# Parskatt/RoMa

Hardware: AMD Instinct MI355X
Metric: image-pairs/sec, roma_outdoor 560->864, batch=8 per GPU (higher is better)
Workload: dtype bf16; 1 GPU; roma_outdoor match() 560->864, symmetric, upsample_preds, 8 pairs/GPU/step, seeded synthetic weights + N(0,1) images; precision policy of the reference's bf16 timing script: bfloat16 DINOv2 + float16 autocast for VGG / decoder / refiners (ROMA_MIXED), f32 accumulate; precision_policy=mixed, global_batch=8, streams_per_gpu=2, parallelism=single GPU, outputs_finite=True

## Files before the change

### roma_amd/csrc/api.hip

```cpp
#include <algorithm>
#include <mutex>
#include <map>
#include <vector>
#include <dlfcn.h>
#include <string.h>

#include "../../include/roma_hip.h"
#include "attention.h"
#include "conv64.h"
#include "conv_patch.h"
#include "elementwise.h"
#include "gemm.h"
#include "local_corr.h"
#include "pool_proj.h"
#include "model.h"
#include "refiner_block.h"
#include "kde.h"
#include "keypoints.h"
#include "tiny.h"
#include "vit.h"
#include "sampling.h"
#include "essential.h"
#include "model_refine.h"
#include "pose_refine.h"
// ... 60 lines not shown

const char* roma_last_error(void) { return g_err.c_str(); }
const char* roma_version(void) { return "roma_hip 0.3 (gfx950, 16-bit storage = " ROMA_H16_NAME ")"; }
int roma_h16_format(void) { return ROMA_H16_CODE; }
int roma_abi_stamp(void) { return ROMA_ABI_VERSION * 100000 + (int)sizeof(roma_vit_args_t); }
int roma_self_check(void) { return roma::internal_h16_code(); }

int roma_create(const roma_config_t* cfg, roma_handle_t* out) {
  ROMA_REQUIRE(cfg && out, "roma_create: null argument");
  ROMA_REQUIRE(cfg->coarse_h > 0 && cfg->coarse_w > 0 && cfg->coarse_h % 14 == 0 && cfg->coarse_w % 14 == 0,
               "Needs to be multiple of 14 for backbone");
  ROMA_REQUIRE(cfg->coarse_h >= 16 && cfg->coarse_w >= 16, "roma_create: coarse resolution too small for the stride-16 pyramid");
  ROMA_REQUIRE(cfg->upsample_h >= 0 && cfg->upsample_w >= 0 && (cfg->upsample_h == 0 || (cfg->upsample_h >= 16 && cfg->upsample_w >= 16)),
               "roma_create: bad upsample resolution");
  ROMA_REQUIRE(cfg->max_batch >= 1, "roma_create: max_batch must be >= 1");
  if (cfg->precision == ROMA_MIXED) {
    ROMA_REQUIRE(ROMA_H16_CODE == ROMA_F16, "ROMA_MIXED: load libroma_hip_f16.so (it runs DINOv2 through libroma_hip.so)");
  } else if (dt_code(cfg->precision) < 0) {
    return ROMA_ERR_ARG;
  }
  int ndev = 0;
  ROMA_CHECK_HIP(hipGetDeviceCount(&ndev));
  ROMA_REQUIRE(cfg->device >= 0 && cfg->device < ndev, "roma_create: no such HIP device (the HIP path has no CPU fallback)");
  roma_model* h = new roma_model();
  h->m.cfg = *cfg;
  *out = h;
  return 0;
}

int roma_set_tensor(roma_handle_t h, const char* name, int ndim, const int64_t* shape, const void* data, int is_int64) {
  ROMA_REQUIRE(h, "roma_set_tensor: null handle");
  return h->m.set_tensor(name, ndim, shape, data, is_int64);
}

int roma_finalize(roma_handle_t h) {
  ROMA_REQUIRE(h, "roma_finalize: null handle");
  return h->m.finalize();
}

int roma_set_option(roma_handle_t h, const char* key, int value) {
  ROMA_REQUIRE(h && key, "roma_set_option: null argument");
  const std::string k(key);
  if (k == "symmetric") h->m.cfg.symmetric = value ? 1 : 0;
  else if (k == "upsample_preds") {
    ROMA_REQUIRE(!value || h->m.cfg.upsample_h > 0, "roma_set_option: handle was created without an upsample resolution");
    h->m.cfg.upsample_preds = value ? 1 : 0;
  } else if (k == "attenuate_cert") h->m.cfg.attenuate_cert = value ? 1 : 0;
  else if (k == "debug") h->m.debug = value != 0;
  else if (k == "fuse_refiner_blocks") h->m.fuse_refiner_blocks = value != 0;
  else if (k == "compose_out_conv") h->m.compose_out_conv = value != 0;
  else if (k == "vit_bf16_residual") h->m.vit_bf16_residual = value != 0;
  else if (k == "dual_stream") h->m.n_streams = value != 0 ? 2 : 1;
  else if (k == "trace") h->m.trace_on = value != 0;
  else if (k == "streams") {
    ROMA_REQUIRE(value >= 1 && value <= Model::MAX_STREAMS, "roma_set_option: streams must be 1..4");
    h->m.n_streams = value;
  }
  else {
    set_error("roma_set_option: unknown key " + k);
    return ROMA_ERR_ARG;
  }
  return 0;
}

int roma_set_option_f(roma_handle_t h, const char* key, double value) {
  ROMA_REQUIRE(h && key, "roma_set_option_f: null argument");
  const std::string k(key);
  if (k == "coarse_scale_factor") {
    ROMA_REQUIRE(value >= 0.0, "roma_set_option_f: coarse_scale_factor must be >= 0 (0 = derive from the handle's resolution)");
    h->m.coarse_scale_factor = value;
  } else {
    set_error("roma_set_option_f: unknown key " + k);
    return ROMA_ERR_ARG;
  }
  return 0;
}

int roma_match(roma_handle_t h, int B, const float* im_a, const float* im_b, const float* im_a_hr, const float* im_b_hr,
               float* warp_out, float* cert_out, void* stream) {
  ROMA_REQUIRE(h, "roma_match: null handle");
  return h->m.match(B, im_a, im_b, im_a_hr, im_b_hr, warp_out, cert_out, S(stream));
}

int roma_forward(roma_handle_t h, int B, const float* im_a, const float* im_b, const roma_forward_args_t* a, void* stream) {
  ROMA_REQUIRE(h, "roma_forward: null handle");
  return h->m.forward(B, im_a, im_b, a, S(stream));
}

long roma_debug_fetch(roma_handle_t h, const char* name, void* dst_host, long nbytes) {
  if (!h || !name) return ROMA_ERR_ARG;
  auto it = h->m.dbg.find(name);
  if (it == h->m.dbg.end()) {
    set_error(std::string("roma_debug_fetch: no such stage: ") + name);
    return ROMA_ERR_ARG;
  }
  if (!dst_host) return (long)it->second.second;
  if ((size_t)nbytes < it->second.second) {
    set_error("roma_debug_fetch: destination too small");
    return ROMA_ERR_ARG;
  }
  if (hipSetDevice(h->m.cfg.device) != hipSuccess || hipDeviceSynchronize() != hipSuccess) return ROMA_ERR_HIP;
  if (hipMemcpy(dst_host, it->second.first, it->second.second, hipMemcpyDeviceToHost) != hipSuccess) return ROMA_ERR_HIP;
  return (long)it->second.second;
}

int roma_debug_inject(roma_handle_t h, const char* name, const void* src_host, long nbytes) {
// ... 443 lines not shown
```

### roma_amd/csrc/model.h

```cpp
#pragma once
#include <stdlib.h>

#include <map>
#include <mutex>
#include <string>
#include <vector>

#include "../../include/roma_hip.h"
#include "common.h"

namespace roma {

extern std::mutex g_peer_mutex;

struct HostTensor {
  std::vector<int64_t> shape;
  std::vector<float> data;
  long numel() const {
    long n = 1;
    for (auto d : shape) n *= d;
    return n;
  }
};

// ... 47 lines not shown
    if (off > peak) peak = off;
    return p;
  }
  size_t mark() const { return off; }
  void release(size_t m) { off = m; }
};

class Model {
 public:
  static constexpr int MAX_STREAMS_DECL = 4;
  roma_config_t cfg{};
  int act_dt = 0;
  bool mixed = false;
  bool pack_as_bf16 = false;
  void* peer_lib = nullptr;
  int (*peer_vit_forward)(const roma_vit_args_t*, void*) = nullptr;
  bool finalized = false;
  bool debug = false;
  bool compose_out_conv = !(getenv("ROMA_COMPOSE_OUT") && atoi(getenv("ROMA_COMPOSE_OUT")) == 0);
  bool vgg_slab_major = !(getenv("ROMA_CONV_KORDER") && atoi(getenv("ROMA_CONV_KORDER")) == 0) &&
                        !(getenv("ROMA_CONV_PATCH") && atoi(getenv("ROMA_CONV_PATCH")) == 0);
  int vgg_korder[12] = {0};
  bool fuse_refiner_blocks = true;
  bool vit_bf16_residual = true;
  bool trace_on = false;
  static constexpr int TRACE_MAX = 1024;
  unsigned long long* trace_dev[MAX_STREAMS_DECL] = {nullptr};
  std::vector<std::string> trace_names[MAX_STREAMS_DECL];
  int trace_n[MAX_STREAMS_DECL] = {0};
  double coarse_scale_factor = 0.0;
  std::map<std::string, HostTensor> host;

  float *c1_w = nullptr, *c1_b = nullptr;
  Lin vgg[12];
  int vgg_cin[12] = {0}, vgg_cout[12] = {0};
  Lin patch;
  float *cls_tok = nullptr, *pos_emb = nullptr;
  VitBlockW dino[24];
  float *dino_nw = nullptr, *dino_nb = nullptr;
  VitBlockW tdec[5];
  Lin to_out;
  float *gp_w = nullptr, *gp_b = nullptr;
  Lin proj[5];
  RefinerW ref[5];

  Arena arena;
  Arena persist;
  static constexpr int MAX_STREAMS = 4;
  int n_streams = 2, streams_ready = 1;
  size_t side_arena_bytes = 0, side_persist_bytes = 0;
  Arena side_arena[MAX_STREAMS - 1], side_persist[MAX_STREAMS - 1];
  hipStream_t side[MAX_STREAMS - 1] = {nullptr};
  hipEvent_t ev_fork = nullptr, ev_join[MAX_STREAMS - 1] = {nullptr};
  std::vector<void*> owned;
  std::map<std::string, std::pair<void*, size_t>> dbg;
  int dbg_cur_slot = 0;
  std::map<std::string, std::pair<void*, size_t>> inject;
  int debug_inject(const char* name, const void* host, size_t bytes);

  ~Model();
  int set_tensor(const char* name, int ndim, const int64_t* shape, const void* data, int is_int64);
  int finalize();
  int match(int B, const float* ima, const float* imb, const float* ima_hr, const float* imb_hr, float* warp,
            float* cert, hipStream_t st);
  int forward(int B, const float* ima, const float* imb, const roma_forward_args_t* fw, hipStream_t st);

 private:
  int ensure_side_streams(int n);
  int match_streams(int B, const float* ima, const float* imb, const float* ima_hr, const float* imb_hr, float* warp,
                    float* cert, hipStream_t st);
  int check_contract();
  int pack_weights();
  int load_peer();
  int match_impl(int B, const float* ima, const float* imb, const float* ima_hr, const float* imb_hr, float* warp,
                 float* cert, hipStream_t st, bool dry, Arena& arena, Arena& persist, const roma_forward_args_t* fw = nullptr);
  int dbg_save(const char* name, const void* p, size_t bytes, hipStream_t st);
  template <typename F> int upload_f32(const std::vector<float>& v, F** out);
  int upload_act(const std::vector<float>& v, void** out);
  int make_lin(const std::vector<float>& w, const std::vector<float>* b, int N, int K, Lin* out);
};

int gp_posterior(const void* pf, long ldf, int act_dt, int B, bool symmetric, int th, int tw, const float* gp_w,
                 const float* gp_b, float* mu, long ld_mu, Arena& arena, hipStream_t st, bool dry);

int cholesky_solve_t(float* A, float* Rt, float* LT, float* Linv, float* LinvT, int n, int d, int batch, hipStream_t st,
                     long strideA = 0, long strideR = 0);

}
```

### roma_amd/csrc/model.hip

```cpp
#include "model.h"

#include <dlfcn.h>
#include <math.h>
#include <stdlib.h>
#include <string.h>

#include <algorithm>
#include <atomic>
#include <set>

#include "attention.h"
#include "conv64.h"
#include "pool_proj.h"
#include "elementwise.h"
#include "gemm.h"
#include "local_corr.h"
#include "refiner_block.h"
#include "vit.h"

namespace roma {

std::mutex g_peer_mutex;
extern void* g_peer_lib;
extern int g_mixed_handles;

static const int VGG_IDX[12] = {0, 3, 7, 10, 14, 17, 20, 23, 27, 30, 33, 36};
static const int VGG_CH[12] = {64, 64, 128, 128, 256, 256, 256, 256, 512, 512, 512, 512};
static const char* SCALES[5] = {"16", "8", "4", "2", "1"};
static const int SCALE_INT[5] = {16, 8, 4, 2, 1};
static const int PROJ_CIN[5] = {1024, 512, 256, 128, 64};
static const int PROJ_COUT[5] = {512, 512, 256, 64, 9};
static const int REF_EMB[5] = {128, 64, 32, 16, 6};
static const int REF_RAD[5] = {7, 3, 2, 0, 0};

Model::~Model() {
  for (int i = 0; i < MAX_STREAMS - 1; ++i) {
    if (side[i]) (void)hipStreamDestroy(side[i]);
    if (ev_join[i]) (void)hipEventDestroy(ev_join[i]);
  }
  if (ev_fork) (void)hipEventDestroy(ev_fork);
  for (void* p : owned) (void)hipFree(p);
  for (auto& kv : dbg) (void)hipFree(kv.second.first);
  for (auto& kv : inject) (void)hipFree(kv.second.first);
  if (peer_lib) {
    std::lock_guard<std::mutex> lk(g_peer_mutex);
    --g_mixed_handles;
  }
}


int Model::load_peer() {
  static void* lib = nullptr;
  static int (*fwd)(const roma_vit_args_t*, void*) = nullptr;
  std::lock_guard<std::mutex> lk(g_peer_mutex);
  if (!lib) {
    ROMA_REQUIRE(roma_h16_format() == ROMA_F16, "ROMA_MIXED is a mode of the binary16 build (libroma_hip_f16.so)");
    Dl_info info;
    ROMA_REQUIRE(dladdr(reinterpret_cast<void*>(&roma_vit_forward), &info) && info.dli_fname, "ROMA_MIXED: cannot locate this library");
    std::string path(info.dli_fname);
    const size_t slash = path.find_last_of('/');
    path = (slash == std::string::npos ? std::string("") : path.substr(0, slash + 1)) + "libroma_hip.so";
    void* l = dlopen(path.c_str(), RTLD_NOW | RTLD_LOCAL | RTLD_DEEPBIND);
    if (!l) {
      set_error("ROMA_MIXED: cannot load the bfloat16 library " + path + ": " + (dlerror() ? dlerror() : "?"));
      return ROMA_ERR_STATE;
    }
    auto fmt = reinterpret_cast<int (*)(void)>(dlsym(l, "roma_h16_format"));
    auto self = reinterpret_cast<int (*)(void)>(dlsym(l, "roma_self_check"));
    auto abi = reinterpret_cast<int (*)(void)>(dlsym(l, "roma_abi_stamp"));
    auto f = reinterpret_cast<int (*)(const roma_vit_args_t*, void*)>(dlsym(l, "roma_vit_forward"));
    std::string why;
    if (!fmt || !f || !self || !abi) why = "it does not export roma_h16_format / roma_self_check / roma_abi_stamp / roma_vit_forward (an older build)";
    else if (fmt() != ROMA_BF16) why = "it is not the bfloat16 build";
    else if (abi() != roma_abi_stamp()) why = "its ABI stamp " + std::to_string(abi()) + " differs from this library's " + std::to_string(roma_abi_stamp()) + " (stale build: roma_vit_args_t would be misread)";
    else if (self() != ROMA_BF16) why = "its internal calls resolve into another library (symbol interposition: link both builds with -Wl,-Bsymbolic)";
    if (!why.empty()) {
      dlclose(l);
      set_error("ROMA_MIXED: " + path + " cannot serve as the bfloat16 sibling: " + why);
      return ROMA_ERR_STATE;
    }
    lib = l;
    fwd = f;
    g_peer_lib = l;
  }
  if (!peer_lib) ++g_mixed_handles;
  peer_lib = lib;
  peer_vit_forward = fwd;
  return 0;
}

int Model::debug_inject(const char* name, const void* host, size_t bytes) {
  ROMA_REQUIRE(name, "roma_debug_inject: null name");
  const std::string k(name);
// ... 400 lines not shown
          for (int k = 0; k < r.Cp; ++k) {
            const float wv = cw[(size_t)o * r.Cp + k];
            const float hi = bf16_to_f32(f32_to_bf16(wv));
            hl[(size_t)o * r.Cp + k] = hi;
            hl[(size_t)(4 + o) * r.Cp + k] = wv - hi;
          }
          fb[o] = cb[o];
        }
        if (int rc = upload_act(hl, &r.ocf_w)) return rc;
        if (int rc = upload_f32(fb, &r.ocf_b)) return rc;
      }
    }
  }
  return 0;
}

int Model::finalize() {
  ROMA_REQUIRE(!finalized, "roma_finalize: already finalized");
  ROMA_CHECK_HIP(hipSetDevice(cfg.device));
  if (int rc = check_contract()) return rc;
  act_dt = cfg.precision == ROMA_F32 ? DT_F32 : DT_BF16;
  mixed = cfg.precision == ROMA_MIXED;
  if (mixed)
    if (int rc = load_peer()) return rc;
  if (int rc = pack_weights()) return rc;
  host.clear();
  arena.dry = persist.dry = true;
  arena.peak = persist.peak = 0;
  const int keep_sym = cfg.symmetric, keep_up = cfg.upsample_preds;
  cfg.symmetric = 1;
  cfg.upsample_preds = cfg.upsample_h > 0 ? 1 : 0;
  int rc = match_impl(cfg.max_batch, nullptr, nullptr, nullptr, nullptr, nullptr, nullptr, nullptr, true, arena, persist);
  Arena plan, plan_p;
  if (!rc && cfg.max_batch >= 2)
    rc = match_impl(cfg.max_batch / 2, nullptr, nullptr, nullptr, nullptr, nullptr, nullptr, nullptr, true, plan, plan_p);
  cfg.symmetric = keep_sym;
  cfg.upsample_preds = keep_up;
  if (rc) return rc;
  side_arena_bytes = plan.peak + 4096;
  side_persist_bytes = plan_p.peak + 4096;
  arena.cap = arena.peak + 4096;
  persist.cap = persist.peak + 4096;
  ROMA_CHECK_HIP(hipMalloc((void**)&arena.base, arena.cap));
  owned.push_back(arena.base);
  ROMA_CHECK_HIP(hipMalloc((void**)&persist.base, persist.cap));
  owned.push_back(persist.base);
  ROMA_CHECK_HIP(hipMemset(persist.base, 0, persist.cap));
  ROMA_CHECK_HIP(hipMemset(arena.base, 0, arena.cap));
  arena.dry = persist.dry = false;
  finalized = true;
  return 0;
}

int Model::ensure_side_streams(int n) {
  for (int i = streams_ready - 1; i + 1 < n; ++i) {
    Arena &a = side_arena[i], &p = side_persist[i];
    a.cap = side_arena_bytes;
    p.cap = side_persist_bytes;
    ROMA_CHECK_HIP(hipMalloc((void**)&a.base, a.cap));
    owned.push_back(a.base);
    ROMA_CHECK_HIP(hipMalloc((void**)&p.base, p.cap));
    owned.push_back(p.base);
    ROMA_CHECK_HIP(hipMemset(p.base, 0, p.cap));
    ROMA_CHECK_HIP(hipMemset(a.base, 0, a.cap));
    ROMA_CHECK_HIP(hipDeviceSynchronize());
    a.dry = p.dry = false;
    ROMA_CHECK_HIP(hipStreamCreateWithFlags(&side[i], hipStreamNonBlocking));
    ROMA_CHECK_HIP(hipEventCreateWithFlags(&ev_join[i], hipEventDisableTiming));
    if (!ev_fork) ROMA_CHECK_HIP(hipEventCreateWithFlags(&ev_fork, hipEventDisableTiming));
    streams_ready = i + 2;
  }
  return 0;
}

static const int g_dbg_dual_slot = getenv("ROMA_DEBUG_DUAL_SLOT") ? atoi(getenv("ROMA_DEBUG_DUAL_SLOT")) : -1;

int Model::dbg_save(const char* name, const void* p, size_t bytes, hipStream_t st) {
  if (!debug) return 0;
  if (g_dbg_dual_slot >= 0) {
    static const std::string only = std::string(",") + (getenv("ROMA_DEBUG_ONLY") ? getenv("ROMA_DEBUG_ONLY") : "") + ",";
    if (dbg_cur_slot != g_dbg_dual_slot || only.find(std::string(",") + name + ",") == std::string::npos) return 0;
  }
  auto it = dbg.find(name);
  if (it == dbg.end() || it->second.second != bytes) {
    if (it != dbg.end()) (void)hipFree(it->second.first);
    void* q = nullptr;
    ROMA_CHECK_HIP(hipMalloc(&q, bytes));
    dbg[name] = {q, bytes};
    it = dbg.find(name);
  }
  ROMA_CHECK_HIP(hipMemcpyAsync(it->second.first, p, bytes, hipMemcpyDeviceToDevice, st));
  return 0;
}

int Model::match(int B, const float* ima, const float* imb, const float* ima_hr, const float* imb_hr, float* warp,
                 float* cert, hipStream_t st) {
  ROMA_REQUIRE(finalized, "roma_match: call roma_finalize first");
  ROMA_REQUIRE(B >= 1 && B <= cfg.max_batch, "roma_match: batch size out of range (max_batch)");
  ROMA_REQUIRE(ima && imb && warp && cert, "roma_match: null image / output pointer");
  if (cfg.upsample_preds) {
    ROMA_REQUIRE(cfg.upsample_h > 0, "roma_match: upsample_preds set but the handle has no upsample resolution");
    ROMA_REQUIRE(ima_hr && imb_hr, "roma_match: upsample_preds requires im_A_high_res and im_B_high_res");
  }
  ROMA_CHECK_HIP(hipSetDevice(cfg.device));
  return match_streams(B, ima, imb, ima_hr, imb_hr, warp, cert, st);
}

int Model::forward(int B, const float* ima, const float* imb, const roma_forward_args_t* fw, hipStream_t st) {
  ROMA_REQUIRE(finalized, "roma_forward: call roma_finalize first");
  ROMA_REQUIRE(B >= 1 && B <= cfg.max_batch, "roma_forward: batch size out of range (max_batch)");
  ROMA_REQUIRE(ima && imb && fw, "roma_forward: null image / argument pointer");
  if (fw->upsample) {
    ROMA_REQUIRE(cfg.upsample_h > 0, "roma_forward: upsample pass on a handle without an upsample resolution");
    ROMA_REQUIRE(fw->seed_flow && fw->seed_cert && fw->seed_h > 0 && fw->seed_w > 0,
                 "roma_forward: the upsample pass needs batch[\"corresps\"] (seed_flow / seed_cert)");
  }
  ROMA_CHECK_HIP(hipSetDevice(cfg.device));
  return match_impl(B, ima, imb, nullptr, nullptr, nullptr, nullptr, st, false, arena, persist, fw);
}

int Model::match_streams(int B, const float* ima, const float* imb, const float* ima_hr, const float* imb_hr, float* warp,
                         float* cert, hipStream_t st) {
  static const int env_streams = getenv("ROMA_STREAMS") ? atoi(getenv("ROMA_STREAMS")) : 0;
  static const bool serial_env = getenv("ROMA_STREAMS_SERIAL") && atoi(getenv("ROMA_STREAMS_SERIAL")) != 0;
  const int ns = (debug && g_dbg_dual_slot < 0) ? 1 : std::min(std::min(env_streams > 0 ? env_streams : n_streams, (int)MAX_STREAMS), B);
  if (ns <= 1) return match_impl(B, ima, imb, ima_hr, imb_hr, warp, cert, st, false, arena, persist);
  if (int rc = ensure_side_streams(ns)) return rc;
  const size_t im_lo = (size_t)3 * cfg.coarse_h * cfg.coarse_w, im_hi = (size_t)3 * cfg.upsample_h * cfg.upsample_w;
  const int Ho = cfg.upsample_preds ? cfg.upsample_h : cfg.coarse_h, Wo = cfg.upsample_preds ? cfg.upsample_w : cfg.coarse_w;
  const size_t px = (size_t)Ho * Wo * (cfg.symmetric ? 2 : 1);
  ROMA_CHECK_HIP(hipEventRecord(ev_fork, st));
  int rc = 0, b0 = 0;
  for (int i = 0; i < ns; ++i) {
    const int bi = B / ns + (i < B % ns ? 1 : 0);
    hipStream_t si = i == 0 ? st : side[i - 1];
    if (i > 0) ROMA_CHECK_HIP(hipStreamWaitEvent(si, ev_fork, 0));
    if (i > 0 && serial_env) {
      hipStream_t sp = i == 1 ? st : side[i - 2];
      ROMA_CHECK_HIP(hipEventRecord(ev_join[i - 1], sp));
      ROMA_CHECK_HIP(hipStreamWaitEvent(si, ev_join[i - 1], 0));
    }
    if (!rc)
      rc = match_impl(bi, ima + b0 * im_lo, imb + b0 * im_lo, ima_hr ? ima_hr + b0 * im_hi : nullptr,
                      imb_hr ? imb_hr + b0 * im_hi : nullptr, warp + b0 * px * 4, cert + b0 * px, si, false,
                      i == 0 ? arena : side_arena[i - 1], i == 0 ? persist : side_persist[i - 1]);
    b0 += bi;
  }
  for (int i = 1; i < ns; ++i) {
    (void)hipEventRecord(ev_join[i - 1], side[i - 1]);
    (void)hipStreamWaitEvent(st, ev_join[i - 1], 0);
  }
  return rc;
}

int g_pool_proj = -1;
int g_gp_col = -1;
int cholesky_solve_t(float* A, float* Rt, float* LT, float* Linv, float* LinvT, int n, int d, int batch, hipStream_t st,
                     long strideA, long strideR) {
  ROMA_REQUIRE(n % 64 == 0 && n > 0 && d % 4 == 0, "cholesky_solve: n must be a multiple of 64, d of 4");
  const int nblk = n / 64;
  const long sA = strideA > 0 ? strideA : (long)n * n, sR = strideR > 0 ? strideR : (long)d * n, sL = (long)nblk * 4096;
  const long sLT = (long)n * n;
  static const bool aug_env = !(getenv("ROMA_GP_AUG") && atoi(getenv("ROMA_GP_AUG")) == 0);
  const bool aug = aug_env && Rt == A + (long)n * n && (batch == 1 || (sA == sR && sA >= (long)(n + d) * n));
  const int extra = aug ? d : 0;
  static const bool col_env = !(getenv("ROMA_GP_COL") && atoi(getenv("ROMA_GP_COL")) == 0);
  const bool col = aug && (g_gp_col >= 0 ? g_gp_col != 0 : col_env) && d >= 64 && d % 64 == 0;
  static std::atomic<unsigned> solve_epoch{0};
  const unsigned epoch = col ? ++solve_epoch : 0u;
  for (int k = 0; k < nblk && col; ++k)
    if (int rc = chol_col_launch(A, n, sA, LT, sLT, n, d, Linv, LinvT, k, nblk, batch, epoch, st)) return rc;
  if (col)
    if (int rc = chol_col_restore_launch(A, n, sA, LT, sLT, n, batch, st)) return rc;
  for (int k = 0; k < nblk && !col; ++k) {
    if (int rc = chol_diag_launch(A, n, sA, Linv, LinvT, k, nblk, batch, st)) return rc;
    const int mrem = n - (k + 1) * 64;
    if (mrem + extra <= 0) break;
    GemmArgs g;
    g.A = A + (long)(k + 1) * 64 * n + k * 64; g.lda = n; g.sA = sA;
    g.W = Linv + (long)k * 4096; g.ldw = 64; g.sW = sL;
// ... 109 lines not shown
    g.nx = norms + (long)j0 * n; g.ny = g.nx; g.sNx = n; g.sNy = n; g.inv_t = 1.0f / 0.2f; g.diag_add = 0.1f;
    GP_RUN(gemm_launch(g, st));
  }
  GP_RUN(pad_identity_launch(Kyy + (long)j0 * saug, npad, saug, n, npad, nj, st));
  if (!dry && npad != n) ROMA_CHECK_HIP(hipMemsetAsync(Kxy, 0, (size_t)ndp * n * npad * 4, st));
  for (int half = 0; half < (symmetric ? 2 : 1); ++half) {
    GemmArgs g;
    const int i0 = half * B, s0 = (i0 + shift) % nimg;
    g.A = off(pf, (long)i0 * n * ldf); g.lda = ldf; g.sA = (long)n * ldf;
    g.W = off(pf, (long)s0 * n * ldf); g.ldw = ldf; g.sW = (long)n * ldf;
    g.C = Kxy + (long)i0 * n * npad; g.ldc = npad; g.sC = (long)n * npad;
    g.M = n; g.N = n; g.K = 512; g.batch = B; g.in_dt = act_dt; g.out_dt = DT_F32; g.mode = EPI_COSK;
    g.nx = norms + (long)i0 * n; g.ny = norms + (long)s0 * n; g.sNx = n; g.sNy = n; g.inv_t = 1.0f / 0.2f;
    GP_RUN(gemm_launch(g, st));
  }
  GP_RUN(gp_basis_launch(gp_w, gp_b, Rt + (long)j0 * saug, 512, th, tw, npad, st, nj, saug));
  GP_RUN(cholesky_solve_t(Kyy + (long)j0 * saug, Rt + (long)j0 * saug, LT + (long)j0 * npad * npad,
                          Linv + (long)j0 * nblk * 4096, LinvT + (long)j0 * nblk * 4096, npad, 512, nj, st, saug, saug));
  for (int half = 0; half < (symmetric ? 2 : 1); ++half) {
    GemmArgs g;
    const int i0 = half * B, s0 = (i0 + shift) % nimg;
    g.A = Kxy + (long)i0 * n * npad; g.lda = npad; g.sA = (long)n * npad;
    g.W = Rt + (long)s0 * saug; g.ldw = npad; g.sW = saug;
    g.C = mu + (long)i0 * n * ld_mu; g.ldc = ld_mu; g.sC = (long)n * ld_mu;
    g.M = n; g.N = 512; g.K = npad; g.batch = B;
    GP_RUN(gemm_launch(g, st));
  }
  return 0;
}
#undef GP_RUN

#define RUN(expr)                 \
  do {                            \
    if (!dry) {                   \
      int _rc = (expr);           \
      if (_rc) return _rc;        \
    }                             \
  } while (0)

int Model::match_impl(int B, const float* ima, const float* imb, const float* ima_hr, const float* imb_hr,
                      float* warp_out, float* cert_out, hipStream_t st, bool dry, Arena& arena, Arena& persist,
                      const roma_forward_args_t* fw) {
  const size_t esz = act_dt == DT_F32 ? 4 : 2;
  const int nimg = 2 * B;
  const bool sym = fw ? fw->symmetric != 0 : cfg.symmetric != 0;
  const int ndp = sym ? 2 * B : B;
  const int shift = B;
  arena.reset();
  persist.reset();
  auto AL = [&](size_t elems, size_t es) { return arena.alloc(elems * es); };
  const int tslot = (&arena == &this->arena) ? 0 : (int)(&arena - side_arena) + 1;
  dbg_cur_slot = tslot;
  const bool tracing = trace_on && !dry;
  if (tracing) {
    if (!trace_dev[tslot]) {
      ROMA_CHECK_HIP(hipMalloc((void**)&trace_dev[tslot], TRACE_MAX * sizeof(unsigned long long)));
      owned.push_back(trace_dev[tslot]);
    }
    ROMA_CHECK_HIP(hipMemsetAsync(trace_dev[tslot], 0, TRACE_MAX * sizeof(unsigned long long), st));
    trace_n[tslot] = 0;
  }
  auto CK = [&](const std::string& name, const void* p, size_t bytes) -> int {
    if (!tracing) return 0;
    if (trace_n[tslot] >= TRACE_MAX) return 0;
    const int k = trace_n[tslot]++;
    if ((int)trace_names[tslot].size() <= k) trace_names[tslot].push_back(name);
    else trace_names[tslot][k] = name;
    return checksum_launch(p, bytes, trace_dev[tslot] + k, st);
  };
  auto off = [&](void* p, long elems) -> void* { return static_cast<char*>(p) + elems * (long)esz; };

  const int th = cfg.coarse_h / 14, tw = cfg.coarse_w / 14, T = th * tw;
  const int Nd = T + 1, Npd = (int)round_up(Nd, 128), Npt = (int)round_up(T, 128);
  const size_t qkv_elems = std::max((size_t)nimg * 16 * Npd * 64, (size_t)ndp * 8 * Npt * 128);
  void* qbuf = persist.alloc(qkv_elems * esz);
  void* kbuf = persist.alloc(qkv_elems * esz);
  void* vtbuf = persist.alloc(qkv_elems * esz);

  float* cert16_keep = (float*)AL((size_t)ndp * T, 4);
  const int Hfin = cfg.upsample_preds ? cfg.upsample_h : cfg.coarse_h;
  const int Wfin = cfg.upsample_preds ? cfg.upsample_w : cfg.coarse_w;
  float *pp_flow[2][2] = {{nullptr, nullptr}, {nullptr, nullptr}}, *pp_cert[2][2] = {{nullptr, nullptr}, {nullptr, nullptr}};
  for (int ps = 0; ps < ((cfg.upsample_preds || (fw && fw->upsample)) ? 2 : 1); ++ps) {
    const size_t px = (size_t)ndp * (ps ? cfg.upsample_h : cfg.coarse_h) * (ps ? cfg.upsample_w : cfg.coarse_w);
    for (int i = 0; i < 2; ++i) {
      pp_flow[ps][i] = (float*)AL(px * 2, 4);
      pp_cert[ps][i] = (float*)AL(px, 4);
    }
  }
  float *flow_p1 = nullptr, *cert_p1 = nullptr;
  float *flow_fin = nullptr, *cert_fin = nullptr;

  auto vit_block = [&](const VitBlockW& w, void* x, int x_dt, long rows, int Bn, int N, int npad, int heads, int hd, float eps,
                       void* ln, void* ao, void* hid) -> int {
    VitScratch sc;
    sc.ln = ln; sc.ao = ao; sc.hid = hid; sc.q = qbuf; sc.k = kbuf; sc.vt = vtbuf;
    RUN(vit_block_run(w.pub(), x, x_dt, rows, Bn, N, npad, heads, hd, eps, act_dt, sc, st));
    return 0;
  };

  const int pass0 = fw ? (fw->upsample ? 1 : 0) : 0, pass1 = fw ? pass0 + 1 : (cfg.upsample_preds ? 2 : 1);
  for (int pass = pass0; pass < pass1; ++pass) {
    const bool up = pass == 1;
    const int H = up ? cfg.upsample_h : cfg.coarse_h, W = up ? cfg.upsample_w : cfg.coarse_w;
    const float* imA = (up && !fw) ? ima_hr : ima;
    const float* imB = (up && !fw) ? imb_hr : imb;
    const size_t pass_mark = arena.mark();
    void* feat[5] = {nullptr};
    const int fh[4] = {H, H / 2, H / 4, H / 8}, fw_[4] = {W, W / 2, W / 4, W / 8};
    const int fc[4] = {64, 128, 256, 512};
    for (int l = 0; l < 4; ++l) feat[l] = AL((size_t)nimg * fh[l] * fw_[l] * fc[l], esz);
    static const bool pp_env = !(getenv("ROMA_POOL_PROJ") && atoi(getenv("ROMA_POOL_PROJ")) == 0);
    void* pf_pre[2] = {nullptr, nullptr};
    const int pp_si[2] = {4, 3};
    bool pp_on[2];
    for (int l = 0; l < 2; ++l) {
      const RefinerW& rr = ref[pp_si[l]];
      const int ldf_l = (int)round_up(rr.Cf, 8);
      pp_on[l] = (g_pool_proj >= 0 ? g_pool_proj != 0 : pp_env) && fh[l] >= 2 && fw_[l] >= 2 &&
                 pool_proj_supported(fc[l], rr.Cf, ldf_l, act_dt) && proj[pp_si[l]].b != nullptr;
      if (pp_on[l] || dry) pf_pre[l] = AL((size_t)nimg * fh[l] * fw_[l] * ldf_l, esz);
      if (!pp_on[l] && !dry) pf_pre[l] = nullptr;
    }
    {
      const size_t enc_mark = arena.mark();
      void* t0 = AL((size_t)nimg * H * W * 64, esz);
      void* t1 = AL((size_t)nimg * (H / 2) * (W / 2) * 64, esz);
      static const int c64_env = getenv("ROMA_CONV64") ? atoi(getenv("ROMA_CONV64")) : 7;
      void* col1 = AL((size_t)nimg * H * W * 32, esz);
      if (act_dt == DT_BF16 && ((g_conv64_mode >= 0 ? g_conv64_mode : c64_env) & 4) && (long)3 * H * W < (1l << 23)) {
        RUN(conv3x3_c3_bf16_launch(imA, vgg[0].w, vgg[0].b, t0, B, H, W, st));
        RUN(conv3x3_c3_bf16_launch(imB, vgg[0].w, vgg[0].b, off(t0, (long)B * H * W * 64), B, H, W, st));
      } else {
        RUN(im2col3x3_c3_launch(imA, col1, B, H, W, act_dt, st));
        RUN(im2col3x3_c3_launch(imB, off(col1, (long)B * H * W * 32), B, H, W, act_dt, st));
        GemmArgs g;
        g.A = col1; g.lda = 32; g.W = vgg[0].w; g.ldw = vgg[0].ldw; g.C = t0; g.ldc = 64;
        g.M = nimg * H * W; g.N = 64; g.K = 32; g.k_alg = 27; g.in_dt = act_dt; g.out_dt = act_dt; g.bias = vgg[0].b; g.act = ACT_RELU;
        RUN(gemm_launch(g, st));
      }
      auto conv = [&](int li, const void* in, void* out, int h, int w) -> int {
        GemmArgs g;
        g.A = in; g.W = vgg[li].w; g.ldw = vgg[li].ldw; g.C = out; g.ldc = vgg_cout[li];
        g.M = nimg * h * w; g.N = vgg_cout[li]; g.K = 9 * vgg_cin[li];
        g.in_dt = act_dt; g.out_dt = act_dt; g.bias = vgg[li].b; g.act = ACT_RELU;
        g.conv_h = h; g.conv_w = w; g.conv_c = vgg_cin[li]; g.conv_korder = vgg_korder[li];
        RUN(gemm_launch(g, st));
        return 0;
      };
      auto pool = [&](int l, const void* in, void* out) -> int {
        if (pp_on[l]) {
          const int si_ = pp_si[l];
          RUN(pool_proj_launch(in, out, pf_pre[l], proj[si_].w, proj[si_].ldw, proj[si_].b, ref[si_].Cf, (int)round_up(ref[si_].Cf, 8),
                               nimg, fh[l], fw_[l], fc[l], act_dt, st));
        } else {
          RUN(maxpool2x2_launch(in, out, nimg, fh[l], fw_[l], fc[l], act_dt, st));
        }
        return 0;
      };
      if (int rc = conv(1, t0, feat[0], H, W)) return rc;
      if (int rc = pool(0, feat[0], t1)) return rc;
      if (int rc = conv(2, t1, t0, H / 2, W / 2)) return rc;
      if (int rc = conv(3, t0, feat[1], H / 2, W / 2)) return rc;
      if (int rc = pool(1, feat[1], t1)) return rc;
      if (int rc = conv(4, t1, t0, H / 4, W / 4)) return rc;
      if (int rc = conv(5, t0, t1, H / 4, W / 4)) return rc;
      if (int rc = conv(6, t1, t0, H / 4, W / 4)) return rc;
      if (int rc = conv(7, t0, feat[2], H / 4, W / 4)) return rc;
      RUN(maxpool2x2_launch(feat[2], t1, nimg, H / 4, W / 4, 256, act_dt, st));
      if (int rc = conv(8, t1, t0, H / 8, W / 8)) return rc;
      if (int rc = conv(9, t0, t1, H / 8, W / 8)) return rc;
      if (int rc = conv(10, t1, t0, H / 8, W / 8)) return rc;
      if (int rc = conv(11, t0, feat[3], H / 8, W / 8)) return rc;
      arena.release(enc_mark);
    }
    for (int l = 0; l < 4; ++l)
      if (int rc = CK((up ? "p2_feat" : "p1_feat") + std::to_string(1 << l), feat[l], (size_t)nimg * fh[l] * fw_[l] * fc[l] * esz)) return rc;
    if (fw && !dry)
      for (int l = 0; l < 4; ++l)
        if (fw->feat[4 - l])
          ROMA_CHECK_HIP(hipMemcpyAsync(fw->feat[4 - l], feat[l], (size_t)nimg * fh[l] * fw_[l] * fc[l] * esz, hipMemcpyDeviceToDevice, st));
    if (debug && !dry && !up) {
      for (int l = 0; l < 4; ++l) {
        const std::string nm = "feat" + std::to_string(1 << l);
        if (int rc = dbg_save(nm.c_str(), feat[l], (size_t)nimg * fh[l] * fw_[l] * fc[l] * esz, st)) return rc;
      }
    }
    const long rows_d = (long)nimg * Nd, rows_t = (long)ndp * T;
    void *ln = nullptr, *ao = nullptr, *hid = nullptr;
    if (!up) {
      feat[4] = AL((size_t)nimg * T * 1024, esz);
      const long rmax = std::max(rows_d, rows_t);
      ln = AL((size_t)rmax * 1024, esz);
      ao = AL((size_t)rmax * 1024, esz);
      hid = AL((size_t)rmax * 4096, esz);
      const size_t dmark = arena.mark();
      void* col = AL((size_t)nimg * T * patch.ldw, esz);
      float* pt = (float*)AL((size_t)nimg * T * 1024, 4);
      float* x = (float*)AL((size_t)rows_d * 1024, 4);
      static const bool res_f32_env = getenv("ROMA_VIT_RES_F32") && atoi(getenv("ROMA_VIT_RES_F32")) != 0;
      void* xs = nullptr;
      if (act_dt == DT_BF16) xs = AL((size_t)rows_d * 1024, 2);
      void* feat_vit = feat[4];
      if (mixed) feat_vit = AL((size_t)nimg * T * 1024, 2);
      if (!dry) {
        roma_vit_block_t blk[24];
        for (int i = 0; i < 24; ++i) blk[i] = dino[i].pub();
        roma_vit_args_t va{};
        va.B = B; va.H = H; va.W = W;
        va.act = act_dt == DT_F32 ? ROMA_F32 : (mixed ? ROMA_BF16 : roma_h16_format());
        va.bf16_residual = act_dt == DT_BF16 && vit_bf16_residual && !res_f32_env;
        va.im_a = imA; va.im_b = imB;
        va.patch_w = patch.w; va.patch_b = patch.b; va.patch_ldw = patch.ldw;
        va.cls_tok = cls_tok; va.pos_emb = pos_emb;
        va.blocks = blk; va.nblocks = 24;
        va.norm_w = dino_nw; va.norm_b = dino_nb;
        va.col = col; va.pt = pt; va.x = x; va.xs = xs; va.ln = ln; va.ao = ao; va.hid = hid;
        va.q = qbuf; va.k = kbuf; va.vt = vtbuf;
        va.feat_out = feat_vit;
        if (mixed) {
          if (int rc = peer_vit_forward(&va, st)) {
            set_error("ROMA_MIXED: roma_vit_forward of the bfloat16 library failed");
            return rc;
          }
          RUN(convert_from_bf16_launch(feat_vit, feat[4], (long)nimg * T * 1024, st));
        } else {
          RUN(vit_forward(va, st));
        }
      }
      arena.release(dmark);
      if (int rc = CK("feat16", feat[4], (size_t)nimg * T * 1024 * esz)) return rc;
      if (debug && !dry)
        if (int rc = dbg_save("feat16", feat[4], (size_t)nimg * T * 1024 * esz, st)) return rc;
      if (fw && !dry && fw->feat[0])
        ROMA_CHECK_HIP(hipMemcpyAsync(fw->feat[0], feat[4], (size_t)nimg * T * 1024 * esz, hipMemcpyDeviceToDevice, st));
    }

    float *flow = pp_flow[pass][0], *cert = pp_cert[pass][0], *flow_alt = pp_flow[pass][1], *cert_alt = pp_cert[pass][1];
    int ch = 0, cw = 0;
    if (up) {
      ch = H / 8; cw = W / 8;
      if (fw) {
        RUN(resize_bilinear_launch(fw->seed_flow, flow, ndp, fw->seed_h, fw->seed_w, ch, cw, 2, st));
        RUN(resize_bilinear_launch(fw->seed_cert, cert, ndp, fw->seed_h, fw->seed_w, ch, cw, 1, st));
      } else {
        RUN(resize_bilinear_launch(flow_p1, flow, ndp, cfg.coarse_h, cfg.coarse_w, ch, cw, 2, st));
        RUN(resize_bilinear_launch(cert_p1, cert, ndp, cfg.coarse_h, cfg.coarse_w, ch, cw, 1, st));
      }
    }
    double scale_factor = sqrt((double)H * (double)W / (560.0 * 560.0));
    if (!up && coarse_scale_factor > 0.0) scale_factor = coarse_scale_factor;
    if (fw && fw->scale_factor > 0.0) scale_factor = fw->scale_factor;
    for (int si = up ? 1 : 0; si < 5; ++si) {
      const int ins = SCALE_INT[si];
      const int hs = ins == 16 ? th : H / ins, ws = ins == 16 ? tw : W / ins;
      const long hw = (long)hs * ws;
      const RefinerW& r = ref[si];
      const size_t smark = arena.mark();
      const int ldf = (int)round_up(r.Cf, 8);
      const int lvl = ins == 16 ? 4 : (ins == 8 ? 3 : (ins == 4 ? 2 : (ins == 2 ? 1 : 0)));
      const bool pf_ready = lvl < 2 && pp_on[lvl];
      void* pf = pf_ready ? pf_pre[lvl] : AL((size_t)nimg * hw * ldf, esz);
      if (!pf_ready) {
        GemmArgs g;
        g.A = feat[lvl]; g.lda = PROJ_CIN[si]; g.W = proj[si].w; g.ldw = proj[si].ldw; g.C = pf; g.ldc = ldf;
        g.M = (int)(nimg * hw); g.N = r.Cf; g.K = PROJ_CIN[si]; g.in_dt = act_dt; g.out_dt = act_dt; g.bias = proj[si].b;
        RUN(gemm_launch(g, st));
      }
      const std::string tp = std::string(up ? "p2_s" : "p1_s") + SCALES[si];
      if (int rc = CK(tp + "_proj", pf, (size_t)nimg * hw * ldf * esz)) return rc;
      if (ins == 16) {
        if (debug && !dry)
          if (int rc = dbg_save("proj16", pf, (size_t)nimg * hw * ldf * esz, st)) return rc;
        const size_t gmark = arena.mark();
        float* tokens = (float*)AL((size_t)rows_t * 1024, 4);
        const size_t gmark2 = arena.mark();
        if (int rc = gp_posterior(pf, ldf, act_dt, B, sym, th, tw, gp_w, gp_b, tokens, 1024, arena, st, dry)) return rc;
        arena.release(gmark2);
        RUN(copy2d_launch(pf, ldf, act_dt, tokens + 512, 1024, DT_F32, rows_t, 512, st));
        if (debug && !dry)
          if (int rc = dbg_save("tokens16", tokens, (size_t)rows_t * 1024 * 4, st)) return rc;
        for (int i = 0; i < 5; ++i)
          if (int rc = vit_block(tdec[i], tokens, DT_F32, rows_t, ndp, T, Npt, 8, 128, 1e-5f, ln, ao, hid)) return rc;
        const int ldl = 4104;
        float* logits = (float*)AL((size_t)rows_t * ldl, 4);
        const void* zin = tokens;
        if (act_dt != DT_F32) {
          RUN(copy2d_launch(tokens, 1024, DT_F32, ln, 1024, act_dt, rows_t, 1024, st));
          zin = ln;
        }
        {
          GemmArgs g;
          g.A = zin; g.lda = 1024; g.W = to_out.w; g.ldw = to_out.ldw; g.C = logits; g.ldc = ldl;
          g.M = (int)rows_t; g.N = to_out.N; g.K = 1024; g.in_dt = act_dt; g.out_dt = DT_F32; g.bias = to_out.b;
          RUN(gemm_launch(g, st));
        }
        if (debug && !dry)
          if (int rc = dbg_save("logits16", logits, (size_t)rows_t * ldl * 4, st)) return rc;
        if (int rc = CK(tp + "_tokens_gp", tokens, (size_t)rows_t * 1024 * 4)) return rc;
        if (int rc = CK(tp + "_logits", logits, (size_t)rows_t * ldl * 4)) return rc;
        RUN(cls_to_flow_launch(logits, ldl, flow, cert, rows_t, st));
        if (int rc = CK(tp + "_gm_flow", flow, (size_t)rows_t * 2 * 4)) return rc;
        ch = th; cw = tw;
        if (debug && !dry) {
          if (int rc = dbg_save("gm_flow16_own", flow, (size_t)rows_t * 2 * 4, st)) return rc;
          auto inj = [&](const char* nm, float* dst, size_t bytes) -> int {
            auto it = inject.find(nm);
            if (it == inject.end()) return 0;
            ROMA_REQUIRE(it->second.second == bytes, "roma_debug_inject: injected stage has the wrong size for this batch");
            ROMA_CHECK_HIP(hipMemcpyAsync(dst, it->second.first, bytes, hipMemcpyDeviceToDevice, st));
            return 0;
          };
          if (int rc = inj("gm_flow16", flow, (size_t)rows_t * 2 * 4)) return rc;
          if (int rc = inj("gm_cert16", cert, (size_t)rows_t * 4)) return rc;
        }
        if (debug && !dry) {
          if (int rc = dbg_save("gm_flow16", flow, (size_t)rows_t * 2 * 4, st)) return rc;
          if (int rc = dbg_save("gm_cert16", cert, (size_t)rows_t * 4, st)) return rc;
        }
        arena.release(gmark);
      }
      {
        const long M = (long)ndp * hw;
        void* d0 = AL((size_t)M * r.Cp, esz);
        void* d1 = AL((size_t)M * r.Cp, esz);
        RefinerInputArgs ia;
        ia.feat = pf; ia.ldf = ldf; ia.flow = flow; ia.d = d0; ia.ldd = r.Cp; ia.emb_w = r.emb_w; ia.emb_b = r.emb_b;
        ia.B = ndp; ia.H = hs; ia.W = ws; ia.C = r.Cf; ia.E = r.E; ia.Kcorr = r.K; ia.nimg = nimg; ia.shift = shift;
        ia.disp_scale = (float)(40.0 / 32.0 * scale_factor); ia.dt = act_dt;
        if (tracing)
          if (int rc = CK(tp + "_flow_before", flow, (size_t)M * 2 * 4)) return rc;
// ... 60 lines not shown
            composed = true;
            break;
          }
          if (fused) {
            RUN(refiner_block_launch(dcur, dalt, r.dw_w[b], r.dw_b[b], r.pw[b].w, r.pw[b].ldw, r.pw[b].b, ndp, hs, ws,
                                     r.Cp, act_dt, st));
            std::swap(dcur, dalt);
            if (int rc = CK(tp + "_blk" + std::to_string(b), dcur, (size_t)M * r.Cp * esz)) return rc;
            continue;
          }
          if (fuse_refiner_blocks && !dry && refiner_block_wide_supported(r.Cp, act_dt)) {
            const int rcw = refiner_block_wide_try_launch(dcur, dalt, r.dw_w[b], r.dw_b[b], r.pw[b].w, r.pw[b].ldw, r.pw[b].b, ndp,
                                                          hs, ws, r.Cp, act_dt, st);
            if (rcw < 0) return rcw;
            if (rcw == 0) {
              std::swap(dcur, dalt);
              if (int rc = CK(tp + "_blk" + std::to_string(b), dcur, (size_t)M * r.Cp * esz)) return rc;
              continue;
            }
          }
          RUN(dwconv5x5_launch(dcur, dalt, r.dw_w[b], r.dw_b[b], ndp, hs, ws, r.Cp, act_dt, st));
          if (int rc = CK(tp + "_dw" + std::to_string(b), dalt, (size_t)M * r.Cp * esz)) return rc;
          GemmArgs g;
          g.A = dalt; g.lda = r.Cp; g.W = r.pw[b].w; g.ldw = r.pw[b].ldw; g.C = dcur; g.ldc = r.Cp;
          g.M = (int)M; g.N = r.Cp; g.K = r.Cp; g.in_dt = act_dt; g.out_dt = act_dt; g.bias = r.pw[b].b;
          g.n_alg = g.k_alg = r.C;
          RUN(gemm_launch(g, st));
          if (int rc = CK(tp + "_blk" + std::to_string(b), dcur, (size_t)M * r.Cp * esz)) return rc;
        }
        const float sx = (float)ins / (4.0f * (float)W), sy = (float)ins / (4.0f * (float)H);
        if (!final_done)
          RUN(refiner_out_launch(dcur, r.Cp, act_dt, composed ? r.oc_w : r.out_w, composed ? r.oc_b : r.out_b, flow, cert, M, r.Cp,
                                 sx, sy, st));
        if (int rc = CK(tp + "_flow", flow, (size_t)M * 2 * 4)) return rc;
        if (int rc = CK(tp + "_cert", cert, (size_t)M * 4)) return rc;
      }
      if (debug && !dry) {
        const std::string pfx = std::string("p") + (up ? "2" : "1");
        if (int rc = dbg_save((pfx + "_flow" + SCALES[si]).c_str(), flow, (size_t)ndp * hw * 2 * 4, st)) return rc;
        if (int rc = dbg_save((pfx + "_cert" + SCALES[si]).c_str(), cert, (size_t)ndp * hw * 4, st)) return rc;
      }
      if (fw && !dry) {
        if (fw->flow[si]) ROMA_CHECK_HIP(hipMemcpyAsync(fw->flow[si], flow, (size_t)ndp * hw * 2 * 4, hipMemcpyDeviceToDevice, st));
        if (fw->cert[si]) ROMA_CHECK_HIP(hipMemcpyAsync(fw->cert[si], cert, (size_t)ndp * hw * 4, hipMemcpyDeviceToDevice, st));
      }
      if (ins == 16) {
        const long nkeep = (long)ndp * hw;
        if (nkeep % 4 == 0) {
          RUN(copy2d_launch(cert, nkeep, DT_F32, cert16_keep, nkeep, DT_F32, 1, (int)nkeep, st));
        } else if (!dry) {
          ROMA_CHECK_HIP(hipMemcpyAsync(cert16_keep, cert, (size_t)nkeep * 4, hipMemcpyDeviceToDevice, st));
        }
      }
      arena.release(smark);
      if (ins != 1) {
        const int nh = H / (ins / 2), nw = W / (ins / 2);
        RUN(resize_bilinear_launch(flow, flow_alt, ndp, hs, ws, nh, nw, 2, st));
        RUN(resize_bilinear_launch(cert, cert_alt, ndp, hs, ws, nh, nw, 1, st));
        std::swap(flow, flow_alt);
        std::swap(cert, cert_alt);
        if (int rc = CK(tp + "_flow_up", flow, (size_t)ndp * nh * nw * 2 * 4)) return rc;
        ch = nh; cw = nw;
      }
    }
    (void)ch; (void)cw;
    flow_fin = flow; cert_fin = cert;
    if (!up) { flow_p1 = flow; cert_p1 = cert; }
    arena.release(pass_mark);
  }
  if (!dry && (arena.overflow || persist.overflow)) {
    arena.overflow = persist.overflow = false;
    set_error("roma_match / roma_forward: the workspace planned by roma_finalize is too small for this call (an option that "
              "changes the buffer plan was switched after roma_finalize); the results of this call are invalid");
    return -5;
  }
  if (fw) return 0;
  FinalArgs fa;
  fa.flow = flow_fin;
  fa.cert = cert_fin;
  fa.cert16 = cfg.attenuate_cert ? cert16_keep : nullptr;
  fa.warp = warp_out; fa.certainty = cert_out;
  fa.B = B; fa.H = Hfin; fa.W = Wfin; fa.h16 = th; fa.w16 = tw; fa.symmetric = cfg.symmetric;
  RUN(final_epilogue_launch(fa, st));
  if (int rc = CK("final_warp", warp_out, (size_t)B * Hfin * Wfin * (cfg.symmetric ? 2 : 1) * 4 * 4)) return rc;
  if (int rc = CK("final_cert", cert_out, (size_t)B * Hfin * Wfin * (cfg.symmetric ? 2 : 1) * 4)) return rc;
  return 0;
}

}
```

Measured before the change: 106.4 image-pairs/s.

## Overlap coarse GP posterior with VGG encoder on an auxiliary stream

In the first (coarse) pass, the VGG encoder now runs after DINOv2, and the scale-16 projection and GP posterior are hoisted ahead of it. The GP posterior is launched on a per-slot auxiliary stream so it can run concurrently with the VGG convolutions, joined back with events. The arena layout is rearranged so GP and VGG scratch are disjoint, and a runtime check guards that. This costs extra streams and events and more arena planning complexity. It is enabled by default only when at most two streams are in use and debug, trace and profiling are off.

```diff
diff --git a/roma_amd/csrc/api.hip b/roma_amd/csrc/api.hip
--- a/roma_amd/csrc/api.hip
+++ b/roma_amd/csrc/api.hip
@@ -136,6 +136,7 @@
   else if (k == "vit_bf16_residual") h->m.vit_bf16_residual = value != 0;
   else if (k == "dual_stream") h->m.n_streams = value != 0 ? 2 : 1;
   else if (k == "trace") h->m.trace_on = value != 0;
+  else if (k == "gp_overlap") h->m.gp_overlap = value != 0;
   else if (k == "streams") {
     ROMA_REQUIRE(value >= 1 && value <= Model::MAX_STREAMS, "roma_set_option: streams must be 1..4");
     h->m.n_streams = value;
diff --git a/roma_amd/csrc/model.h b/roma_amd/csrc/model.h
--- a/roma_amd/csrc/model.h
+++ b/roma_amd/csrc/model.h
@@ -123,6 +123,10 @@
   Arena side_arena[MAX_STREAMS - 1], side_persist[MAX_STREAMS - 1];
   hipStream_t side[MAX_STREAMS - 1] = {nullptr};
   hipEvent_t ev_fork = nullptr, ev_join[MAX_STREAMS - 1] = {nullptr};
+  bool gp_overlap = true;
+  bool gp_overlap_ns_ok = false;
+  hipStream_t aux[MAX_STREAMS] = {nullptr};
+  hipEvent_t aux_fork[MAX_STREAMS] = {nullptr}, aux_join[MAX_STREAMS] = {nullptr};
   std::vector<void*> owned;
   std::map<std::string, std::pair<void*, size_t>> dbg;
   int dbg_cur_slot = 0;
@@ -137,7 +141,8 @@
   int forward(int B, const float* ima, const float* imb, const roma_forward_args_t* fw, hipStream_t st);
 
  private:
-  int ensure_side_streams(int n);
+  int ensure_side_streams(int n, bool want_aux);
+  bool gp_overlap_wanted() const;
   int match_streams(int B, const float* ima, const float* imb, const float* ima_hr, const float* imb_hr, float* warp,
                     float* cert, hipStream_t st);
   int check_contract();
diff --git a/roma_amd/csrc/model.hip b/roma_amd/csrc/model.hip
--- a/roma_amd/csrc/model.hip
+++ b/roma_amd/csrc/model.hip
@@ -39,6 +39,11 @@
     if (ev_join[i]) (void)hipEventDestroy(ev_join[i]);
   }
   if (ev_fork) (void)hipEventDestroy(ev_fork);
+  for (int i = 0; i < MAX_STREAMS; ++i) {
+    if (aux[i]) (void)hipStreamDestroy(aux[i]);
+    if (aux_fork[i]) (void)hipEventDestroy(aux_fork[i]);
+    if (aux_join[i]) (void)hipEventDestroy(aux_join[i]);
+  }
   for (void* p : owned) (void)hipFree(p);
   for (auto& kv : dbg) (void)hipFree(kv.second.first);
   for (auto& kv : inject) (void)hipFree(kv.second.first);
@@ -545,7 +550,21 @@
   return 0;
 }
 
-int Model::ensure_side_streams(int n) {
+int Model::ensure_side_streams(int n, bool want_aux) {
+  static const bool aux_prio_env = getenv("ROMA_GP_OVERLAP_PRIO") && atoi(getenv("ROMA_GP_OVERLAP_PRIO")) != 0;
+  for (int i = 0; want_aux && i < n && i < MAX_STREAMS; ++i) {
+    if (aux[i]) continue;
+    if (!aux_fork[i]) ROMA_CHECK_HIP(hipEventCreateWithFlags(&aux_fork[i], hipEventDisableTiming));
+    if (!aux_join[i]) ROMA_CHECK_HIP(hipEventCreateWithFlags(&aux_join[i], hipEventDisableTiming));
+    int least = 0, greatest = 0;
+    if (aux_prio_env && hipDeviceGetStreamPriorityRange(&least, &greatest) == hipSuccess && greatest != least) {
+      if (hipStreamCreateWithPriority(&aux[i], hipStreamNonBlocking, greatest) != hipSuccess) {
+        (void)hipGetLastError();
+        aux[i] = nullptr;
+      }
+    }
+    if (!aux[i]) ROMA_CHECK_HIP(hipStreamCreateWithFlags(&aux[i], hipStreamNonBlocking));
+  }
   for (int i = streams_ready - 1; i + 1 < n; ++i) {
     Arena &a = side_arena[i], &p = side_persist[i];
     a.cap = side_arena_bytes;
@@ -612,13 +631,19 @@
   return match_impl(B, ima, imb, nullptr, nullptr, nullptr, nullptr, st, false, arena, persist, fw);
 }
 
+bool Model::gp_overlap_wanted() const {
+  static const int ovl_env = getenv("ROMA_GP_OVERLAP") ? atoi(getenv("ROMA_GP_OVERLAP")) : -1;
+  return (ovl_env >= 0 ? ovl_env != 0 : gp_overlap) && !debug && !trace_on && !prof_enabled();
+}
+
 int Model::match_streams(int B, const float* ima, const float* imb, const float* ima_hr, const float* imb_hr, float* warp,
                          float* cert, hipStream_t st) {
   static const int env_streams = getenv("ROMA_STREAMS") ? atoi(getenv("ROMA_STREAMS")) : 0;
   static const bool serial_env = getenv("ROMA_STREAMS_SERIAL") && atoi(getenv("ROMA_STREAMS_SERIAL")) != 0;
   const int ns = (debug && g_dbg_dual_slot < 0) ? 1 : std::min(std::min(env_streams > 0 ? env_streams : n_streams, (int)MAX_STREAMS), B);
+  gp_overlap_ns_ok = ns <= 2;
+  if (int rc = ensure_side_streams(ns, gp_overlap_ns_ok && gp_overlap_wanted())) return rc;
   if (ns <= 1) return match_impl(B, ima, imb, ima_hr, imb_hr, warp, cert, st, false, arena, persist);
-  if (int rc = ensure_side_streams(ns)) return rc;
   const size_t im_lo = (size_t)3 * cfg.coarse_h * cfg.coarse_w, im_hi = (size_t)3 * cfg.upsample_h * cfg.upsample_w;
   const int Ho = cfg.upsample_preds ? cfg.upsample_h : cfg.coarse_h, Wo = cfg.upsample_preds ? cfg.upsample_w : cfg.coarse_w;
   const size_t px = (size_t)Ho * Wo * (cfg.symmetric ? 2 : 1);
@@ -834,6 +859,8 @@
   const int tslot = (&arena == &this->arena) ? 0 : (int)(&arena - side_arena) + 1;
   dbg_cur_slot = tslot;
   const bool tracing = trace_on && !dry;
+  const bool ovl = !dry && !fw && gp_overlap_ns_ok && aux[tslot] != nullptr && gp_overlap_wanted();
+  const bool ovl_layout = dry || ovl;
   if (tracing) {
     if (!trace_dev[tslot]) {
       ROMA_CHECK_HIP(hipMalloc((void**)&trace_dev[tslot], TRACE_MAX * sizeof(unsigned long long)));
@@ -904,12 +931,15 @@
       if (pp_on[l] || dry) pf_pre[l] = AL((size_t)nimg * fh[l] * fw_[l] * ldf_l, esz);
       if (!pp_on[l] && !dry) pf_pre[l] = nullptr;
     }
-    {
-      const size_t enc_mark = arena.mark();
-      void* t0 = AL((size_t)nimg * H * W * 64, esz);
-      void* t1 = AL((size_t)nimg * (H / 2) * (W / 2) * 64, esz);
+    const bool hoist = ovl_layout && !up;
+    void *t0 = nullptr, *t1 = nullptr, *col1 = nullptr;
+    auto vgg_alloc = [&]() {
+      t0 = AL((size_t)nimg * H * W * 64, esz);
+      t1 = AL((size_t)nimg * (H / 2) * (W / 2) * 64, esz);
+      col1 = AL((size_t)nimg * H * W * 32, esz);
+    };
+    auto vgg_run = [&]() -> int {
       static const int c64_env = getenv("ROMA_CONV64") ? atoi(getenv("ROMA_CONV64")) : 7;
-      void* col1 = AL((size_t)nimg * H * W * 32, esz);
       if (act_dt == DT_BF16 && ((g_conv64_mode >= 0 ? g_conv64_mode : c64_env) & 4) && (long)3 * H * W < (1l << 23)) {
         RUN(conv3x3_c3_bf16_launch(imA, vgg[0].w, vgg[0].b, t0, B, H, W, st));
         RUN(conv3x3_c3_bf16_launch(imB, vgg[0].w, vgg[0].b, off(t0, (long)B * H * W * 64), B, H, W, st));
@@ -954,6 +984,12 @@
       if (int rc = conv(9, t0, t1, H / 8, W / 8)) return rc;
       if (int rc = conv(10, t1, t0, H / 8, W / 8)) return rc;
       if (int rc = conv(11, t0, feat[3], H / 8, W / 8)) return rc;
+      return 0;
+    };
+    if (!hoist) {
+      const size_t enc_mark = arena.mark();
+      vgg_alloc();
+      if (int rc = vgg_run()) return rc;
       arena.release(enc_mark);
     }
     for (int l = 0; l < 4; ++l)
@@ -970,12 +1006,21 @@
     }
     const long rows_d = (long)nimg * Nd, rows_t = (long)ndp * T;
     void *ln = nullptr, *ao = nullptr, *hid = nullptr;
+    void* pf16 = nullptr;
+    float* tokens16 = nullptr;
+    size_t hoist_mark = 0;
+    const int ldf16 = (int)round_up(ref[0].Cf, 8);
     if (!up) {
       feat[4] = AL((size_t)nimg * T * 1024, esz);
       const long rmax = std::max(rows_d, rows_t);
       ln = AL((size_t)rmax * 1024, esz);
       ao = AL((size_t)rmax * 1024, esz);
       hid = AL((size_t)rmax * 4096, esz);
+      if (hoist) {
+        hoist_mark = arena.mark();
+        pf16 = AL((size_t)nimg * T * ldf16, esz);
+        tokens16 = (float*)AL((size_t)rows_t * 1024, 4);
+      }
       const size_t dmark = arena.mark();
       void* col = AL((size_t)nimg * T * patch.ldw, esz);
       float* pt = (float*)AL((size_t)nimg * T * 1024, 4);
@@ -985,6 +1030,27 @@
       if (act_dt == DT_BF16) xs = AL((size_t)rows_d * 1024, 2);
       void* feat_vit = feat[4];
       if (mixed) feat_vit = AL((size_t)nimg * T * 1024, 2);
+      size_t gp_top = 0, fork_top = 0;
+      if (hoist) {
+        const size_t dino_top = arena.mark();
+        arena.release(dmark);
+        if (int rc = gp_posterior(pf16, ldf16, act_dt, B, sym, th, tw, gp_w, gp_b, tokens16, 1024, arena, st, true)) return rc;
+        gp_top = arena.mark();
+        vgg_alloc();
+        fork_top = arena.mark();
+        if (!dry && (arena.overflow || persist.overflow)) {
+          arena.overflow = persist.overflow = false;
+          set_error("roma_match: the workspace planned by roma_finalize is too small for this call (an option that changes the "
+                    "buffer plan was switched after roma_finalize); nothing was launched");
+          return -5;
+        }
+        auto at = [&](size_t o) { return (arena.dry ? (uintptr_t)0x1000 : (uintptr_t)arena.base) + o; };
+        ROMA_REQUIRE((uintptr_t)tokens16 + (size_t)rows_t * 1024 * 4 <= at(dmark) && at(dmark) <= at(gp_top) &&
+                         at(gp_top) <= (uintptr_t)t0 && (uintptr_t)t0 < (uintptr_t)t1 && (uintptr_t)t1 < (uintptr_t)col1 &&
+                         (uintptr_t)col1 + (size_t)nimg * H * W * 32 * esz <= at(fork_top),
+                     "roma_match: the GP and VGG scratch ranges of the overlapped coarse pass are not disjoint");
+        arena.release(std::max(dino_top, fork_top));
+      }
       if (!dry) {
         roma_vit_block_t blk[24];
         for (int i = 0; i < 24; ++i) blk[i] = dino[i].pub();
@@ -1016,6 +1082,32 @@
         if (int rc = dbg_save("feat16", feat[4], (size_t)nimg * T * 1024 * esz, st)) return rc;
       if (fw && !dry && fw->feat[0])
         ROMA_CHECK_HIP(hipMemcpyAsync(fw->feat[0], feat[4], (size_t)nimg * T * 1024 * esz, hipMemcpyDeviceToDevice, st));
+      if (hoist) {
+        {
+          GemmArgs g;
+          g.A = feat[4]; g.lda = PROJ_CIN[0]; g.W = proj[0].w; g.ldw = proj[0].ldw; g.C = pf16; g.ldc = ldf16;
+          g.M = (int)((long)nimg * T); g.N = ref[0].Cf; g.K = PROJ_CIN[0]; g.in_dt = act_dt; g.out_dt = act_dt; g.bias = proj[0].b;
+          RUN(gemm_launch(g, st));
+        }
+        hipStream_t ax = dry ? st : aux[tslot];
+        if (!dry) {
+          ROMA_CHECK_HIP(hipEventRecord(aux_fork[tslot], st));
+          ROMA_CHECK_HIP(hipStreamWaitEvent(ax, aux_fork[tslot], 0));
+        }
+        int rc = gp_posterior(pf16, ldf16, act_dt, B, sym, th, tw, gp_w, gp_b, tokens16, 1024, arena, ax, dry);
+        if (!rc && arena.mark() != gp_top) {
+          set_error("roma_match: the GP scratch of the overlapped coarse pass left its planned range");
+          rc = -1;
+        }
+        arena.release(fork_top);
+        if (!rc) rc = vgg_run();
+        if (!dry) {
+          (void)hipEventRecord(aux_join[tslot], ax);
+          (void)hipStreamWaitEvent(st, aux_join[tslot], 0);
+        }
+        if (rc) return rc;
+        arena.release(dmark);
+      }
     }
 
     float *flow = pp_flow[pass][0], *cert = pp_cert[pass][0], *flow_alt = pp_flow[pass][1], *cert_alt = pp_cert[pass][1];
@@ -1042,8 +1134,9 @@
       const int ldf = (int)round_up(r.Cf, 8);
       const int lvl = ins == 16 ? 4 : (ins == 8 ? 3 : (ins == 4 ? 2 : (ins == 2 ? 1 : 0)));
       const bool pf_ready = lvl < 2 && pp_on[lvl];
-      void* pf = pf_ready ? pf_pre[lvl] : AL((size_t)nimg * hw * ldf, esz);
-      if (!pf_ready) {
+      const bool hoisted = hoist && ins == 16;
+      void* pf = hoisted ? pf16 : (pf_ready ? pf_pre[lvl] : AL((size_t)nimg * hw * ldf, esz));
+      if (!pf_ready && !hoisted) {
         GemmArgs g;
         g.A = feat[lvl]; g.lda = PROJ_CIN[si]; g.W = proj[si].w; g.ldw = proj[si].ldw; g.C = pf; g.ldc = ldf;
         g.M = (int)(nimg * hw); g.N = r.Cf; g.K = PROJ_CIN[si]; g.in_dt = act_dt; g.out_dt = act_dt; g.bias = proj[si].b;
@@ -1055,10 +1148,12 @@
         if (debug && !dry)
           if (int rc = dbg_save("proj16", pf, (size_t)nimg * hw * ldf * esz, st)) return rc;
         const size_t gmark = arena.mark();
-        float* tokens = (float*)AL((size_t)rows_t * 1024, 4);
-        const size_t gmark2 = arena.mark();
-        if (int rc = gp_posterior(pf, ldf, act_dt, B, sym, th, tw, gp_w, gp_b, tokens, 1024, arena, st, dry)) return rc;
-        arena.release(gmark2);
+        float* tokens = hoisted ? tokens16 : (float*)AL((size_t)rows_t * 1024, 4);
+        if (!hoisted) {
+          const size_t gmark2 = arena.mark();
+          if (int rc = gp_posterior(pf, ldf, act_dt, B, sym, th, tw, gp_w, gp_b, tokens, 1024, arena, st, dry)) return rc;
+          arena.release(gmark2);
+        }
         RUN(copy2d_launch(pf, ldf, act_dt, tokens + 512, 1024, DT_F32, rows_t, 512, st));
         if (debug && !dry)
           if (int rc = dbg_save("tokens16", tokens, (size_t)rows_t * 1024 * 4, st)) return rc;
@@ -1225,7 +1320,7 @@
           ROMA_CHECK_HIP(hipMemcpyAsync(cert16_keep, cert, (size_t)nkeep * 4, hipMemcpyDeviceToDevice, st));
         }
       }
-      arena.release(smark);
+      arena.release(hoisted ? hoist_mark : smark);
       if (ins != 1) {
         const int nh = H / (ins / 2), nw = W / (ins / 2);
         RUN(resize_bilinear_launch(flow, flow_alt, ndp, hs, ws, nh, nw, 2, st));
```

After: 107.2 image-pairs/s (median of 6 runs). Within noise of the previous version (+0.8%).
